# tensorboy/centerpose

Measured on AMD Instinct MI355X. Metric: images/sec end-to-end (backbone+decode), DLA-34 512x512, higher is better.
Workload: dtype f32

## Files before the change

centerpose_amd/csrc/conv3x3_wino24.hip:

```cpp
#include <type_traits>
#include "igemm.h"

#define W24_PH 18
#define W24_PW 18
#define W24_PWP 20
#define W24_KS 16
#define W24_CGS (W24_KS / 4)
#define W24_CG (W24_PH * W24_PWP * 4 + 16)
#define W24_STAGE (W24_CGS * W24_CG)
#define W24_F4 (W24_PH * W24_PW * W24_CGS)
#define W24_SLOTS ((W24_F4 + IG_THREADS - 1) / IG_THREADS)
#define W24_LDR 36
#define W24_RED (16 * 32 * W24_LDR)
#define W24_MAIN (2 * W24_STAGE > W24_RED ? 2 * W24_STAGE : W24_RED)
#define W24_SMEM_FLOATS (W24_MAIN + 16)

typedef float w24_v2 __attribute__((ext_vector_type(2)));
typedef float w24_v4 __attribute__((ext_vector_type(4)));

struct W24Grid {
    int tilesX, tilesY, ntb;
    unsigned mNtb, mTx, mTy;
};
__device__ __forceinline__ int w24_div(int n, int d, unsigned magic) { return d == 1 ? n : (int)__umulhi((unsigned)n, magic); }
__device__ __forceinline__ w24_v4 w24_lds4(const float* p) { return *reinterpret_cast<const w24_v4*>(p); }

__device__ __forceinline__ void w24_output_generic(const ConvArgs& a, float* red, int tid, int b, int y0, int x0, int tile)
{
    const float* const a_res = a.res;
    const bool relu = a.act == CP_ACT_RELU;
    const bool vec_ok = (a.outLd & 3) == 0 && (((size_t)a.out) & 15) == 0 &&
                        (!a_res || ((a.resLd & 3) == 0 && (((size_t)a_res) & 15) == 0));
    const int n4 = tid & 7, n = tile * 32 + n4 * 4;
    const bool nvec = vec_ok && n + 3 < a.Cout;
    w24_v4 sc = {1.f, 1.f, 1.f, 1.f}, sh = {0.f, 0.f, 0.f, 0.f};
    if (nvec) {
        sc = *reinterpret_cast<const w24_v4*>(a.scale + n);
        sh = *reinterpret_cast<const w24_v4*>(a.shift + n);
// ... 104 lines not shown
        const w24_v4 q0 = w24_lds4(rp), q1 = w24_lds4(rp + 128 * W24_LDR), q2 = w24_lds4(rp + 256 * W24_LDR), q3 = w24_lds4(rp + 384 * W24_LDR);
        w24_v4 yv[2];
        yv[0] = (q0 + q1) + q2;
        yv[1] = (q1 - q2) - q3;
#pragma unroll
        for (int aa = 0; aa < 2; ++aa) {
            if (!(okx && oyb + 4 * it + aa < a.H)) continue;
            w24_v4 v = __builtin_elementwise_fma(yv[aa], sc, sh);
            if (a_res) v += rr[it][aa];
            if (relu) v = (w24_v4){cp_relu(v.x), cp_relu(v.y), cp_relu(v.z), cp_relu(v.w)};
            *reinterpret_cast<w24_v4*>(op + (4 * it + aa) * ostep) = v;
        }
    }
}

template <bool FAST>
__device__ __forceinline__ void w24_block(const ConvArgs& a, const W24Grid& gd, int t_, float* smem)
{
    constexpr int CPS = W24_KS / 8;
    const int tid = threadIdx.x, lane = tid & 63, xi = __builtin_amdgcn_readfirstlane(tid >> 6);
    const int h = lane >> 5, m = lane & 31;
    const int NTILES = (a.Cout + 31) >> 5;
    int q_;
    q_ = w24_div(t_, gd.ntb, gd.mNtb); const int nb = t_ - q_ * gd.ntb; t_ = q_;
    q_ = w24_div(t_, gd.tilesX, gd.mTx); const int tx = t_ - q_ * gd.tilesX; t_ = q_;
    q_ = w24_div(t_, gd.tilesY, gd.mTy); const int ty = t_ - q_ * gd.tilesY;
    const int b = q_;
    const int y0 = ty * 16, x0 = tx * 16;
    const int C = a.srcC[0], ld = a.srcLd[0];
    const int KC = C >> 3;
    const float* __restrict__ x = a.src[0];
    const bool interior = y0 >= 1 && y0 + 17 <= a.H && x0 >= 1 && x0 + 17 <= a.W;

    int go[W24_SLOTS], lo[W24_SLOTS];
    bool ok[W24_SLOTS];
#pragma unroll
    for (int s = 0; s < W24_SLOTS; ++s) {
        const int idx = tid + s * IG_THREADS;
        const int pp = idx / W24_CGS, q = idx % W24_CGS;
        const int py = pp / W24_PW, px = pp - py * W24_PW;
        const int gy = y0 - 1 + py, gx = x0 - 1 + px;
        const bool inl = idx < W24_F4;
        ok[s] = inl && gy >= 0 && gy < a.H && gx >= 0 && gx < a.W;
        go[s] = ok[s] ? ((b * a.H + gy) * a.W + gx) * ld + q * 4 : 0;
        lo[s] = inl ? q * W24_CG + (py * W24_PWP + (px ^ ((py >> 1) & 3))) * 4 : -1;
    }
    float4 rg[W24_SLOTS];
    auto stage_load = [&](int c0) __attribute__((always_inline)) {
#pragma unroll
        for (int s = 0; s < W24_SLOTS; ++s) rg[s] = ig_ldg4(x + go[s] + c0);
    };
    auto stage_store = [&](float* buf) __attribute__((always_inline)) {
        if (interior) {
#pragma unroll
            for (int s = 0; s < W24_SLOTS; ++s)
                if ((s + 1) * IG_THREADS <= W24_F4 || lo[s] >= 0) *reinterpret_cast<float4*>(buf + lo[s]) = rg[s];
        } else {
#pragma unroll
            for (int s = 0; s < W24_SLOTS; ++s)
                if ((s + 1) * IG_THREADS <= W24_F4 || lo[s] >= 0) {
                    float4 v = rg[s];
                    if (!ok[s]) v = make_float4(0.f, 0.f, 0.f, 0.f);
// ... 13 lines not shown
    int offA[4], offB[4];
#pragma unroll
    for (int jj = 0; jj < 4; ++jj) { offA[jj] = baseA + ((jj ^ sA) << 2); offB[jj] = baseB + ((jj ^ sB) << 2); }

    int tile = nb;
    if (tile >= NTILES) tile = NTILES - 1;
    const float* ub = a.w + ((size_t)(xi * NTILES + tile) * KC) * 1536 + lane * 4;
    float4 bq[2][6];
    auto load_u = [&](int kc, float4 (&dst)[6]) __attribute__((always_inline)) {
        const int kk = kc < KC ? kc : KC - 1;
#pragma unroll
        for (int nu = 0; nu < 6; ++nu) dst[nu] = ig_ldg4(ub + (size_t)kk * 1536 + nu * 256);
    };

    const int nstage = C / W24_KS;
    stage_load(0);
    load_u(0, bq[0]);
    stage_store(smem);
    if (tid < 4) *reinterpret_cast<float4*>(smem + W24_MAIN + tid * 4) = make_float4(0.f, 0.f, 0.f, 0.f);
    __syncthreads();
    f32x16 acc[6];
    {
        const w24_v4* zp = reinterpret_cast<const w24_v4*>(smem + W24_MAIN);
#pragma unroll
        for (int nu = 0; nu < 6; ++nu)
#pragma unroll
            for (int r4 = 0; r4 < 4; ++r4) {
                w24_v4 z = zp[r4];
                asm volatile("" : "+v"(z));
                acc[nu][4 * r4] = z.x; acc[nu][4 * r4 + 1] = z.y; acc[nu][4 * r4 + 2] = z.z; acc[nu][4 * r4 + 3] = z.w;
            }
    }

// ... 17 lines not shown
                const w24_v2 k4 = {4.f, 4.f}, kn4 = {-4.f, -4.f}, k2 = {2.f, 2.f}, kn2 = {-2.f, -2.f};
                const w24_v2 al = __builtin_elementwise_fma(kn4, tl[2], tl[4]), ah = __builtin_elementwise_fma(kn4, th[2], th[4]);
                const w24_v2 bl = __builtin_elementwise_fma(kn4, tl[1], tl[3]), bh = __builtin_elementwise_fma(kn4, th[1], th[3]);
                const w24_v2 cl = tl[4] - tl[2], chh = th[4] - th[2];
                const w24_v2 fl = tl[3] - tl[1], fh = th[3] - th[1];
                vl[0] = __builtin_elementwise_fma(k4, tl[0] - tl[2], cl); vh[0] = __builtin_elementwise_fma(k4, th[0] - th[2], chh);
                vl[5] = __builtin_elementwise_fma(kn4, fl, tl[5] - tl[3]); vh[5] = __builtin_elementwise_fma(kn4, fh, th[5] - th[3]);
                vl[1] = al + bl; vh[1] = ah + bh;
                vl[2] = al - bl; vh[2] = ah - bh;
                vl[3] = __builtin_elementwise_fma(k2, fl, cl); vh[3] = __builtin_elementwise_fma(k2, fh, chh);
                vl[4] = __builtin_elementwise_fma(kn2, fl, cl); vh[4] = __builtin_elementwise_fma(kn2, fh, chh);
            }
            __builtin_amdgcn_sched_barrier(0);
#pragma unroll
            for (int nu = 0; nu < 6; ++nu) {
                if (nu == 1) {
                    load_u(st * CPS + ch + 1, bq[(ch + 1) & 1]);
                    __builtin_amdgcn_sched_barrier(0);
                }
                if (nu == 3 && ch == 0 && more) {
                    stage_load((st + 1) * W24_KS);
                    __builtin_amdgcn_sched_barrier(0);
                }
                if (nu == 4 && ch == CPS - 1 && more) {
                    stage_store(smem + (BUF ^ 1) * W24_STAGE);
                    __builtin_amdgcn_sched_barrier(0);
                }
                const float4 bb = bq[ch & 1][nu];
                acc[nu] = __builtin_amdgcn_mfma_f32_32x32x2f32(bb.x, vl[nu].x, acc[nu], 0, 0, 0);
                acc[nu] = __builtin_amdgcn_mfma_f32_32x32x2f32(bb.y, vl[nu].y, acc[nu], 0, 0, 0);
                acc[nu] = __builtin_amdgcn_mfma_f32_32x32x2f32(bb.z, vh[nu].x, acc[nu], 0, 0, 0);
                acc[nu] = __builtin_amdgcn_mfma_f32_32x32x2f32(bb.w, vh[nu].y, acc[nu], 0, 0, 0);
            }
            __builtin_amdgcn_sched_barrier(0);
        }
        __syncthreads();
    };
#pragma unroll 1
    for (int st = 0; st < nstage; st += 2) {
        stage(st, std::integral_constant<int, 0>{});
// ... 14 lines not shown

struct W24Group {
    ConvArgs a[4];
    W24Grid gd[4];
    int first[5];
    int n;
};
template <bool FAST>
__global__ __launch_bounds__(IG_THREADS, 2) void conv3x3_wino24_group_kernel(const W24Group g)
{
    extern __shared__ __attribute__((aligned(16))) float smem[];
    const int t = blockIdx.x;
    int k = 0;
    while (k + 1 < g.n && t >= g.first[k + 1]) ++k;
    w24_block<FAST>(g.a[k], g.gd[k], t - g.first[k], smem);
}

static bool w24_fast_epilogue(const ConvArgs& a)
{
    return (a.outLd & 3) == 0 && (a.Cout & 3) == 0 && (((size_t)a.out) & 15) == 0 &&
           (!a.res || ((a.resLd & 3) == 0 && (((size_t)a.res) & 15) == 0)) && (a.act == CP_ACT_NONE || a.act == CP_ACT_RELU) &&
           (long long)a.W * a.outLd * 8 < (1ll << 31) && (long long)a.W * a.resLd * 8 < (1ll << 31);
}

static unsigned w24_magic(int d) { return d <= 1 ? 0u : (unsigned)(((1ull << 32) + (unsigned)d - 1) / (unsigned)d); }

int cp_launch_conv3x3_wino24(const ConvArgs& a, hipStream_t s)
{
    const bool ok = a.nsrc == 1 && a.kh == 3 && a.kw == 3 && a.sy == 1 && a.sx == 1 && a.py == 1 && a.px == 1 &&
                    !a.outNCHW && a.osy == 1 && a.osx == 1 && a.ooy == 0 && a.oox == 0 && a.Ho == a.H && a.Wo == a.W &&
// ... 6 lines not shown
    static CpLdsGuard guard[2];
    {
        const hipError_t e = guard[fast].ensure(fast ? (const void*)conv3x3_wino24_kernel<true> : (const void*)conv3x3_wino24_kernel<false>, smem);
        if (e != hipSuccess) { cp_set_error("conv3x3_winograd24: cannot reserve %d B LDS: %s", smem, hipGetErrorString(e)); return 2; }
    }
    W24Grid gd;
    gd.tilesX = cp_cdiv(a.W, 16); gd.tilesY = cp_cdiv(a.H, 16);
    gd.ntb = (a.Cout + 31) / 32;
    gd.mNtb = w24_magic(gd.ntb); gd.mTx = w24_magic(gd.tilesX); gd.mTy = w24_magic(gd.tilesY);
    const long long grid = (long long)a.B * gd.tilesX * gd.tilesY * gd.ntb;
    const long long dmax = gd.ntb > gd.tilesX ? (gd.ntb > gd.tilesY ? gd.ntb : gd.tilesY) : (gd.tilesX > gd.tilesY ? gd.tilesX : gd.tilesY);
    if (grid * dmax >= (1ll << 32)) { cp_set_error("conv3x3_winograd24: grid %lld too large", grid); return 1; }
    if (fast) hipLaunchKernelGGL(conv3x3_wino24_kernel<true>, dim3((unsigned)grid), dim3(IG_THREADS), smem, s, a, gd);
    else hipLaunchKernelGGL(conv3x3_wino24_kernel<false>, dim3((unsigned)grid), dim3(IG_THREADS), smem, s, a, gd);
    cp_note_kernel(fast ? "conv3x3_wino24_kernel<true>" : "conv3x3_wino24_kernel<false>");
    return 0;
}

int cp_launch_conv3x3_wino24_group(const ConvArgs* a, int n, hipStream_t s)
{
    if (n < 1 || n > 4) { cp_set_error("conv3x3_winograd24_group: 1..4 members (got %d)", n); return 1; }
    W24Group g;
    g.n = n;
    bool fast = true;
    long long total = 0, dmax = 1;
    for (int i = 0; i < n; ++i) {
        const ConvArgs& c = a[i];
        const bool ok = c.nsrc == 1 && c.kh == 3 && c.kw == 3 && c.sy == 1 && c.sx == 1 && c.py == 1 && c.px == 1 &&
                        !c.outNCHW && c.osy == 1 && c.osx == 1 && c.ooy == 0 && c.oox == 0 && c.Ho == c.H && c.Wo == c.W &&
                        c.OH == c.H && c.OW == c.W && c.srcC[0] % 16 == 0 && c.srcLd[0] % 4 == 0 && c.ksplit == 1 &&
// ... 75 lines not shown
```

centerpose_amd/csrc/conv_igemm.hip:

```cpp
#include <cstdlib>
#include "igemm.h"

struct PixSlot {
    int boff;
    int iy0, ix0;
};

template <int BM, int BN, int WAVES_M, int WAVES_N, int MF, bool STEM>
__device__ __forceinline__ void igemm_conv_block(const ConvArgs& a, int tile, int nblocks, float* smem)
{
    using T = IgTile<BM, BN, WAVES_M, WAVES_N, MF>;
    float* As0 = smem;
    float* Bs0 = smem + 2 * T::A_FLOATS;

    const int tid = threadIdx.x, lane = tid & 63, wid = tid >> 6;
    const float* wsub = a.w;
    int pys = a.py, pxs = a.px, ooys = 0, ooxs = 0;
    if (a.nsub > 1) {
        const int per = nblocks / a.nsub, sub = tile / per;
        tile -= sub * per;
        wsub += (size_t)sub * a.ldw * a.K;
        pys -= sub >> 1; pxs -= sub & 1;
        ooys = sub >> 1; ooxs = sub & 1;
    }
// ... 420 lines not shown
                                               float* const* out, void* stream)
{
    CP_CHECK_ARG(d && src && u && scale && shift && res && out && n >= 1 && n <= 4, "conv3x3_winograd24_group: 1..4 members, no null arrays");
    ConvArgs a[4];
    for (int i = 0; i < n; ++i) {
        const float* srcs[1] = {src[i]};
        CP_CHECK_ARG(d[i].nsrc == 1 && !d[i].inNCHW, "conv3x3_winograd24_group: member %d: one NHWC source expected", i);
        if (int rc = conv_args_from_desc(&d[i], srcs, u[i], scale[i], shift[i], res[i], out[i], a[i])) return rc;
        CP_CHECK_ARG(a[i].ksplit == 1, "conv3x3_winograd24_group: no split launches inside a group");
    }
    if (int rc = cp_launch_conv3x3_wino24_group(a, n, (hipStream_t)stream)) return rc;
    CP_CHECK_LAUNCH("conv3x3_wino24_group_kernel");
    return 0;
}

extern "C" int cp_conv3x3_winograd_f32(const cp_conv_desc* d, const float* src, const float* u, const float* scale,
                                       const float* shift, const float* res, float* out, void* stream)
{
    ConvArgs a;
    const float* srcs[1] = {src};
    CP_CHECK_ARG(d && d->nsrc == 1 && !d->inNCHW, "conv3x3_winograd: one NHWC source expected");
    if (int rc = conv_args_from_desc(d, srcs, u, scale, shift, res, out, a)) return rc;
    CP_CHECK_ARG(a.ksplit == 1 || (!res && d->act == CP_ACT_NONE && !d->outNCHW),
                 "conv3x3_winograd: split-C writes raw NHWC partial outputs (no residual, no activation; scale = ones, shift = zeros)");
    const int rc = cp_launch_conv3x3_wino(a, (hipStream_t)stream, d->tile);
    CP_CHECK_ARG(rc >= 0, "conv3x3_winograd: shape not eligible (3x3, stride 1, pad 1, NHWC, C %% 16 == 0)");
    if (rc) return rc;
    CP_CHECK_LAUNCH("conv3x3_wino_kernel");
    return 0;
}
// ... 1 lines not shown
```

centerpose_amd/csrc/igemm.h:

```cpp
#pragma once
#include "common.h"

#define IG_BK 16
#define IG_LDK 20
#define IG_THREADS 256
#define IG_MAX_SRC 4

enum { CP_ACT_NONE = 0, CP_ACT_RELU = 1, CP_ACT_SIGMOID = 2 };

struct ConvArgs {
    const float* src[IG_MAX_SRC];
    int srcC[IG_MAX_SRC];
    int srcLd[IG_MAX_SRC];
    int nsrc, Ctot;
    int B, H, W;
    int Ho, Wo, M;
    int kh, kw, sy, sx, py, px;
    int K;
    const float* w;
    int ldw;
    const float* scale;
    const float* shift;
    const float* res;
    int resLd;
// ... 9 lines not shown
    int omMaskOff;
    int omSigmoid;
    int dily, dilx;
    int ksplit;
    int dg;
    int nsub;
};

int cp_launch_conv3x3_patch(const ConvArgs& a, int in_nchw, hipStream_t s, int variant = 0);
int cp_launch_stem3x3(const ConvArgs& a, hipStream_t s);
int cp_launch_conv3x3_c16(const ConvArgs& a, int in_nchw, hipStream_t s);
int cp_launch_conv3x3_wino(const ConvArgs& a, hipStream_t s, int variant = 0);
int cp_launch_conv3x3_wino24_group(const ConvArgs* a, int n, hipStream_t s);
int cp_launch_head3x3_1x1_w24(const ConvArgs& a, const float* w2, const float* b2, float* out2, int n2, int ld2, int act2, hipStream_t s);
int cp_launch_conv3x3_wino24(const ConvArgs& a, hipStream_t s);
int cp_launch_head3x3_1x1(const ConvArgs& a, const float* w2, const float* b2, float* out2, int n2, int ld2, int act2, hipStream_t s);

int cp_launch_conv_pointwise(const ConvArgs& a, hipStream_t s);
int cp_launch_conv_bf16x3(const ConvArgs& a, int tile, hipStream_t s);

typedef float ig_v4f __attribute__((ext_vector_type(4)));
__device__ __forceinline__ float4 ig_ldg4(const float* p)
{
    const ig_v4f v = *(const __attribute__((address_space(1))) ig_v4f*)(p);
    return make_float4(v.x, v.y, v.z, v.w);
}

__device__ __forceinline__ int ig_xcd_remap(int id, int n)
{
    const int q = n >> 3, r = n & 7, x = id & 7, j = id >> 3;
// ... 212 lines not shown
```

centerpose_amd/csrc/plan_runtime.cpp:

```cpp
#include <cstdio>
#include <cstring>
#include <memory>
#include <string>
#include <vector>
#include "common.h"

extern "C" {
struct cp_conv_desc;
struct cp_dcn_desc;
int cp_abi_version(void);
int cp_conv2d_f32(const cp_conv_desc*, const float* const*, const float*, const float*, const float*, const float*, float*, void*);
int cp_conv3x3_winograd_f32(const cp_conv_desc*, const float*, const float*, const float*, const float*, const float*, float*, void*);
int cp_dcn_v2_f32(const cp_dcn_desc*, const float*, const float*, const float*, const float*, const float*, float*, void*);
int cp_conv3x3_winograd24_group_f32(const cp_conv_desc*, int, const float* const*, const float* const*, const float* const*, const float* const*,
                                    const float* const*, float* const*, void*);
int cp_conv2d_group_f32(const cp_conv_desc*, int, const float* const*, const float* const*, const float* const*, const float* const*,
                        const float* const*, float* const*, void*);
int cp_stem7x7_f32(const float*, const float*, const float*, const float*, float*, int, int, int, int, int, int, int, void*);
int cp_maxpool2d_nhwc_f32(const float*, int, float*, int, int, int, int, int, int, int, int, void*);
int cp_dw_deconv_add_nhwc_f32(const float*, int, const float*, const float*, int, float*, int, int, int, int, int, int, void*);
int cp_sum_up_nhwc_f32(int, const float* const*, const int*, const int*, float*, int, int, int, int, int, int, void*);
int cp_sum_up_group_nhwc_f32(int, const float* const*, const int*, float* const*, int, void*);
int cp_head3x3_1x1_f32(const cp_conv_desc*, const float*, const float*, const float*, const float*, const float*, const float*, float*, int,
                       int, int, void*);
int cp_dwconv2d_nhwc_f32(const float*, int, const float*, const float*, const float*, float*, int, int, int, int, int, int, int, int, int, void*);
int cp_global_avgpool_nhwc_f32(const float*, int, float*, int, int, int, int, void*);
int cp_scale_add_nhwc_f32(const float*, int, const float*, int, const float*, int, float*, int, int, int, int, int, void*);
int cp_shuffle_concat_nhwc_f32(const float*, int, const float*, int, float*, int, long long, int, int, void*);
int cp_multi_pose_decode_f32(const float*, const float*, const float*, const float*, const float*, const float*, int, int, int, int,
                             int, int, float*, float*, int*, void*);
int cp_splitk_reduce_f32(const float*, int, int, int, const float*, const float*, int, float*, int, int, void*);
int cp_sizeof_conv_desc(void);
int cp_sizeof_dcn_desc(void);
int cp_decode_topk_f32(const float*, const float*, int, int, int, int, int, int, float*, int*, void*);
int cp_decode_assign_f32(const float*, const float*, const float*, const float*, const float*, const int*, int, int, int, int, int, float*,
                         void*);
int cp_head_points_f32(const float*, int, const int*, const float*, const float*, const float*, const float*, float*, int, int, int, int, int,
                       int, int, void*);
int cp_flip_merge_pairs_f32(int, const float* const*, float* const*, const int*, int, int, int, int, const int*, void*);
}

namespace {

enum { FN_CONV = 1, FN_WINO = 2, FN_DCN = 3, FN_STEM7 = 4, FN_POOL = 5, FN_UPADD = 6, FN_SUMUP = 7, FN_DWCONV = 8, FN_AVGPOOL = 9,
       FN_SCALEADD = 10, FN_SHUFFLE = 11, FN_HEAD = 12, FN_TOPK = 13, FN_ASSIGN = 14, FN_SPLITK = 15, FN_WINO24G = 16, FN_CONVG = 17, FN_SUMUPG = 18,
       FN_POINTS = 19, FN_FLIPPAIRS = 20 };
enum { REF_NULL = 0, REF_BUF = 1, REF_CONST = 2 };

struct Op {
    uint32_t fn = 0, out_index = 0, stream = 0;
    std::vector<unsigned char> desc;
    std::vector<float*> ptrs;
    std::vector<int> bufid;
    std::vector<int> ints;
};

struct Out { float* p; int shape[4]; int bufid; };

struct ConstPool {
    std::vector<float*> p;
    ~ConstPool() { for (float* q : p) if (q) (void)hipFree(q); }
// ... 82 lines not shown
            return cp_scale_add_nhwc_f32(P[0], I[0], P[1], I[1], P[2], I[2], P[3], I[3], I[4], I[5], I[6], I[7], s);
        case FN_SHUFFLE:
            return cp_shuffle_concat_nhwc_f32(P[0], I[0], P[1], I[1], P[2], I[2], (long long)I[3], I[4], I[5], s);
        case FN_SPLITK:
            return cp_splitk_reduce_f32(P[0], I[0], I[1], I[2], P[1], P[2], I[3], P[3], I[4], I[5], s);
        case FN_TOPK:
            return cp_decode_topk_f32(P[0], P[1], I[0], I[1], I[2], I[3], I[4], I[5], P[2], reinterpret_cast<int*>(P[3]), s);
        case FN_ASSIGN:
            return cp_decode_assign_f32(P[0], P[1], P[2], P[3], P[4], reinterpret_cast<const int*>(P[5]), I[0], I[1], I[2], I[3], I[4], P[6], s);
        case FN_POINTS:
            return cp_head_points_f32(P[0], I[0], reinterpret_cast<const int*>(P[1]), P[2], P[3], P[4], P[5], P[6], I[1], I[2], I[3], I[4], I[5],
                                      I[6], I[7], s);
        case FN_FLIPPAIRS:
            return cp_flip_merge_pairs_f32(I[0], reinterpret_cast<const float* const*>(P.data()), reinterpret_cast<float* const*>(P.data() + 4), I + 5,
                                           I[1], I[2], I[3], I[4], reinterpret_cast<const int*>(P[8]), s);
    }
    cp_set_error("plan: unknown launch function %u", o.fn);
    return 1;
}

bool arity_ok(const Op& o)
{
    switch (o.fn) {
        case FN_CONV: return o.ptrs.size() == 9 && (int)o.desc.size() == cp_sizeof_conv_desc();
        case FN_WINO: return o.ptrs.size() == 6 && (int)o.desc.size() == cp_sizeof_conv_desc();
        case FN_DCN: return o.ptrs.size() == 6 && (int)o.desc.size() == cp_sizeof_dcn_desc();
        case FN_WINO24G: return o.ptrs.size() == 25 && o.ints.size() == 1 && o.ints[0] >= 1 && o.ints[0] <= 4 && (int)o.desc.size() == 4 * cp_sizeof_conv_desc();
        case FN_CONVG: return o.ptrs.size() == 49 && o.ints.size() == 1 && o.ints[0] >= 1 && o.ints[0] <= 8 && (int)o.desc.size() == 8 * cp_sizeof_conv_desc();
        case FN_STEM7: return o.ptrs.size() == 5 && o.ints.size() == 7;
        case FN_POOL: return o.ptrs.size() == 2 && o.ints.size() == 9;
        case FN_UPADD: return o.ptrs.size() == 4 && o.ints.size() == 8;
        case FN_SUMUP: return o.ptrs.size() == 5 && o.ints.size() == 15;
        case FN_SUMUPG: return o.ptrs.size() == 21 && o.ints.size() == 58 && o.ints[0] >= 1 && o.ints[0] <= 4;
        case FN_HEAD: return o.ptrs.size() == 7 && o.ints.size() == 3 && (int)o.desc.size() == cp_sizeof_conv_desc();
        case FN_DWCONV: return o.ptrs.size() == 5 && o.ints.size() == 10;
        case FN_AVGPOOL: return o.ptrs.size() == 2 && o.ints.size() == 5;
        case FN_SCALEADD: return o.ptrs.size() == 4 && o.ints.size() == 8;
        case FN_SHUFFLE: return o.ptrs.size() == 3 && o.ints.size() == 6;
        case FN_SPLITK: return o.ptrs.size() == 4 && o.ints.size() == 6;
        case FN_TOPK: return o.ptrs.size() == 4 && o.ints.size() == 6;
        case FN_ASSIGN: return o.ptrs.size() == 7 && o.ints.size() == 5;
        case FN_POINTS: return o.ptrs.size() == 7 && o.ints.size() == 8;
        case FN_FLIPPAIRS: return o.ptrs.size() == 10 && o.ints.size() == 13 && o.ints[0] >= 1 && o.ints[0] <= 4;
    }
    return false;
}

int run_all(cp_plan* pl, hipStream_t s)
{
    for (const Op& o : pl->ops)
        if (int rc = run_op(o, s)) return rc;
    return 0;
}

struct SchedOp { const Op* op; int stream; int buf_base; };

int run_schedule(const std::vector<SchedOp>& ops, size_t nb, hipStream_t main, hipStream_t side, std::vector<hipEvent_t>& ev)
{
// ... 434 lines not shown
```

centerpose_amd/engine.py:

```python
import os
import warnings
import weakref

import torch

from . import _lib, nets, ops
from .nets import Act


DECODE_TOPK = "decode.nms_topk"
SPARSE_HEADS = ("wh", "hps", "reg", "hp_offset")
FLIP_PEAKS = "flip.merge_peaks"
FLIP_IDX = ((1, 2), (3, 4), (5, 6), (7, 8), (9, 10), (11, 12), (13, 14), (15, 16))


def normalize_state_dict(sd, arch=None):
    out = {}
    for k, v in sd.items():
        if k.startswith("module") and not k.startswith("module_list"):
            k = k[7:]
        out[nets.internal_key(arch, k) if arch is not None else k] = v
    return out


# ... 31 lines not shown
        super().__init__()
        self.dets_only = dets_only
        self.points = None
        self.sd, self.B, self.dev = sd, B, device
        self.const_cache = const_cache if const_cache is not None else {}
        self.pool = BufferPool(device, lambda: len(self.launches))
        if isinstance(sigmoid_heads, bool):
            sigmoid_heads = ("hm", "hm_hp") if sigmoid_heads else ()
        self.sigmoid_heads = tuple(sigmoid_heads)
        self.launches = []
        self.winograd = os.environ.get("CP_WINOGRAD", "1") != "0"
        self.dcn_splitk = os.environ.get("CP_DCN_SPLITK", "1") != "0"
        self.wino_splitc = os.environ.get("CP_WINO_SPLITC", "1") != "0"
        self.conv_splitk = os.environ.get("CP_CONV_SPLITK", "1") != "0"
        self.fuse_heads = os.environ.get("CP_FUSE_HEADS", "1") != "0"
        self._pool_cache = {}
        self.outputs = None

    @property
    def bytes_alloc(self):
        return self.pool.bytes

    def buf(self, H, W, C, split=None):
        Cp = 2 * split[1] if split else ops.round_up(C, 16)
        slot = self.pool.take(self.B * H * W * Cp)
        act = Act(H, W, C, slot[: self.B * H * W * Cp].view(self.B, H, W, Cp), split)
        weakref.finalize(act, self.pool.give, slot)
        return act

    @staticmethod
# ... 178 lines not shown
                outs.append(out)
            self.add("conv", "group:" + chunk[0][1], flops, ops.conv2d_group_launch(recs, slot[:off]))
        return outs

    def emit_maxpool(self, x, k, s, p):
        key = (id(x), k, s, p)
        hit = self._pool_cache.get(key)
        if hit is not None and hit[0]() is x and hit[1]() is not None:
            return hit[1]()
        out = self.buf((x.H + 2 * p - k) // s + 1, (x.W + 2 * p - k) // s + 1, x.C)
        self.add("pool", "maxpool%dx%d" % (k, k), 0, ops.maxpool2d_launch(x.t, out.t, k, s, p))
        self._pool_cache[key] = (weakref.ref(x), weakref.ref(out))
        return out

    def emit_dcn(self, x, conv, bn, co):
        om = self.buf(x.H, x.W, 32)
        wom = ops.pack_conv_weight(self.expand_in(self.w(conv + ".conv_offset_mask.weight"), [x]))
        som, hom = ops.fold_bn(27, None, self.w(conv + ".conv_offset_mask.bias"), self.dev)
        som[27:] = 0.0
        out = self.buf(x.H, x.W, co)
        wp = ops.pack_conv_weight(self.expand_in(self.w(conv + ".weight"), [x]))
        sc, sh = ops.fold_bn(co, self.bn(bn), self.w(conv + ".bias"), self.dev)
        uom = self.wino(wom, x.t.shape[3], 32, key=conv + ".conv_offset_mask", hw=(x.H, x.W))
        if uom is not None:
            self.add_wino(conv + ".conv_offset_mask", 2 * x.H * x.W * 27 * x.C * 9, x.t, wom, uom, som, hom, om.t, 32, ops.ACT_NONE)
        else:
            self.add("conv", conv + ".conv_offset_mask", 2 * x.H * x.W * 27 * x.C * 9,
                     ops.conv2d_launch([x.t], wom, som, hom, om.t, kh=3, kw=3, stride=1, pad=1, cout=32))
        flops = 2 * x.H * x.W * co * x.C * 9
        S = ops.dcn_ksplit(ops.rule_batch(self.B) * x.H * x.W, wp.shape[0]) if self.dcn_splitk else 1
        if S > 1:
            ldw = wp.shape[0]
            ws = self.pool.take(S * self.B * x.H * x.W * ldw)
            wst = ws[: S * self.B * x.H * x.W * ldw].view(S, self.B * x.H * x.W, ldw)
            ones, zeros = self.unit_scale(ldw)
            self.add("dcn", conv, flops, ops.dcn_v2_launch(x.t, om.t, wp, ones, zeros, wst, cout=ldw, om_sigmoid=True, ksplit=S))
            self.add("sum", conv + ".splitk", 0, ops.splitk_reduce_launch(wst, sc, sh, out.t, cout=out.t.shape[3], act=ops.ACT_RELU))
            self.pool.give(ws)
            return out
        self.add("dcn", conv, flops,
                 ops.dcn_v2_launch(x.t, om.t, wp, sc, sh, out.t, cout=out.t.shape[3], om_sigmoid=True, act=ops.ACT_RELU))
        return out

    def emit_up_add(self, x, wname, f, add):
        out = self.buf(x.H * f, x.W * f, x.C)
        wk = ops.pack_dw_deconv_weight(self.w(wname + ".weight"))
        if wk.shape[1] != x.t.shape[3]:
            wk = torch.cat([wk, wk.new_zeros((wk.shape[0], x.t.shape[3] - wk.shape[1]))], 1).contiguous()
        self.add("up", wname, 2 * out.H * out.W * x.C * 4, ops.dw_deconv_add_launch(x.t, wk, add.t, out.t, f))
        return out

    def emit_dwconv(self, x, conv, bn, k, stride, act):
        Ho, Wo = (x.H + 2 * (k // 2) - k) // stride + 1, (x.W + 2 * (k // 2) - k) // stride + 1
        out = self.buf(Ho, Wo, x.C, x.split)
        g, b, mean, var = self.bn(bn)
        scale = g / torch.sqrt(var + ops.BN_EPS)
        shift = b - mean * scale
        wk = ops.pack_dw_weight(self.w(conv + ".weight"))
        wkp = torch.stack([self.expand_vec(row, x) for row in wk], 0).contiguous()
        self.add("dw", conv, 2 * Ho * Wo * x.C * k * k,
                 ops.dwconv2d_launch(x.t, wkp, self.expand_vec(scale, x), self.expand_vec(shift, x), out.t, k, stride, k // 2,
                                     self.act_code(act)))
        return out

# ... 434 lines not shown
        if tuple(images.shape) != tuple(self.input.shape):
            raise ValueError("engine was planned for input %s, got %s" % (tuple(self.input.shape), tuple(images.shape)))
        if images.data_ptr() != self.input.data_ptr():
            self.input.copy_(images)
        if self.use_graph:
            if self.graph is None:
                self.capture()
            self.graph.replay()
        else:
            self.run_eager()
        return self.outputs

    __call__ = forward

    def launch_bytes(self, launches=None):
        grouped = ("cp_conv3x3_winograd24_group_f32", "cp_conv2d_group_f32", "cp_sum_up_group_nhwc_f32", "cp_flip_merge_pairs_f32")
        return [sum(4 * t.numel() for t in (launch.tensors[:-1] if launch.fn in grouped else launch.tensors) if t is not None)
                for _, _, _, launch in (self.launches if launches is None else launches)]

    def profile(self, iters=5):
        torch.cuda.synchronize(self.device)
        self.run_eager()
        nbytes = self.launch_bytes()
        recs = []
        for (kind, name, flops, launch), nb in zip(self.launches, nbytes):
            e0, e1 = torch.cuda.Event(enable_timing=True), torch.cuda.Event(enable_timing=True)
            e0.record()
            for _ in range(iters):
                launch.run()
            e1.record()
            e1.synchronize()
# ... 77 lines not shown
```

centerpose_amd/ops.py:

```python
import ctypes
import os

import torch

from . import _lib

ACT_NONE, ACT_RELU, ACT_SIGMOID, ACT_HSWISH, ACT_HSIGMOID = 0, 1, 2, 3, 4
BN_EPS = 1e-5


class ConvDesc(ctypes.Structure):
    _fields_ = [(n, ctypes.c_int) for n in ("nsrc",)] + [("srcC", ctypes.c_int * 4), ("srcLd", ctypes.c_int * 4)] + \
        [(n, ctypes.c_int) for n in ("B", "H", "W", "Ho", "Wo", "kh", "kw", "sy", "sx", "py", "px", "K", "ldw", "Cout",
                                     "resLd", "outLd", "outNCHW", "OH", "OW", "osy", "osx", "ooy", "oox", "act",
                                     "inNCHW", "tile", "nsub", "ksplit")]


class DcnDesc(ctypes.Structure):
    _fields_ = [(n, ctypes.c_int) for n in ("B", "H", "W", "C", "srcLd", "Ho", "Wo", "kh", "kw", "sy", "sx", "py", "px",
                                            "dily", "dilx", "K", "ldw", "Cout", "omLd", "omSigmoid", "outLd",
                                            "outNCHW", "act", "tile", "ksplit", "dg")]


def round_up(x, m):
# ... 72 lines not shown
    if fn == "cp_shuffle_concat_nhwc_f32":
        return [ptrs[0], ints[0], ptrs[1], ints[1], ptrs[2], ints[2], ctypes.c_longlong(ints[3]), ints[4], ints[5]]
    if fn == "cp_splitk_reduce_f32":
        return [ptrs[0], ints[0], ints[1], ints[2], ptrs[1], ptrs[2], ints[3], ptrs[3], ints[4], ints[5]]
    if fn == "cp_decode_topk_f32":
        return ptrs[:2] + ints + ptrs[2:]
    if fn == "cp_decode_assign_f32":
        return ptrs[:6] + ints + [ptrs[6]]
    if fn == "cp_head_points_f32":
        return [ptrs[0], ints[0]] + ptrs[1:] + ints[1:]
    if fn == "cp_flip_merge_pairs_f32":
        ins = (ctypes.c_void_p * 4)(*[p.value for p in ptrs[:4]])
        outs = (ctypes.c_void_p * 4)(*[p.value for p in ptrs[4:8]])
        meta = (ctypes.c_int * 8)(*ints[5:13])
        return [ints[0], ins, outs, meta] + ints[1:5] + [ptrs[8]]
    raise ValueError("unknown launch function %r" % fn)


FN_IDS = {"cp_conv2d_f32": 1, "cp_conv3x3_winograd_f32": 2, "cp_dcn_v2_f32": 3, "cp_stem7x7_f32": 4,
          "cp_maxpool2d_nhwc_f32": 5, "cp_dw_deconv_add_nhwc_f32": 6, "cp_sum_up_nhwc_f32": 7, "cp_dwconv2d_nhwc_f32": 8,
          "cp_global_avgpool_nhwc_f32": 9, "cp_scale_add_nhwc_f32": 10, "cp_shuffle_concat_nhwc_f32": 11, "cp_head3x3_1x1_f32": 12,
          "cp_decode_topk_f32": 13, "cp_decode_assign_f32": 14, "cp_splitk_reduce_f32": 15, "cp_conv3x3_winograd24_group_f32": 16, "cp_conv2d_group_f32": 17,
          "cp_sum_up_group_nhwc_f32": 18, "cp_head_points_f32": 19,
          "cp_flip_merge_pairs_f32": 20}


def pad_rows(t, ldw):
    Co, K = t.shape
    if Co == ldw:
        return t.contiguous()
    out = torch.zeros((ldw, K), dtype=t.dtype, device=t.device)
    out[:Co] = t
    return out


def pad_vec(v, ldw, fill=0.0):
    out = torch.full((ldw,), fill, dtype=torch.float32, device=v.device)
    out[: v.numel()] = v
    return out
# ... 320 lines not shown
    return out


def pack_dw_deconv_weight(w):
    C, _, k, _ = w.shape
    return w.reshape(C, k * k).t().contiguous().float()


def dw_deconv_add_launch(x, wk, add, out, f):
    B, H, W, C = x.shape
    assert wk.is_contiguous()
    return Launch("cp_dw_deconv_add_nhwc_f32", None, [x, wk, add, out],
                  [_ld(x), _ld(add) if add is not None else 0, _ld(out), B, H, W, C, f])


def dw_deconv_add(x, wk, add, out, f):
    dw_deconv_add_launch(x, wk, add, out, f).run()
    return out


def pack_dw_weight(w):
    C, _, k, _ = w.shape
    return w.reshape(C, k * k).t().contiguous().float()


def dwconv2d_launch(x, wk, scale, shift, out, k, stride, pad, act=ACT_NONE):
    B, H, W, C = x.shape
    assert wk.shape == (k * k, C) and wk.is_contiguous() and scale.numel() >= C and shift.numel() >= C
    return Launch("cp_dwconv2d_nhwc_f32", None, [x, wk, scale, shift, out], [_ld(x), _ld(out), B, H, W, C, k, stride, pad, act])

# ... 162 lines not shown
```

centerpose_amd/plan.py:

```python
import ctypes
import json
import struct

import numpy as np
import torch

from . import _lib, ops

MAGIC = b"CPPLAN04"
MAGIC_V3 = b"CPPLAN03"
MAGIC_V2 = b"CPPLAN02"


def checksum(data):
    mv = memoryview(data).cast("B")
    n = len(mv)
    if n == 0:
        return 2166136261
    buf = (ctypes.c_ubyte * n).from_buffer_copy(mv) if mv.readonly else (ctypes.c_ubyte * n).from_buffer(mv)
    L = _lib.lib()
    L.cp_fnv1a32.restype = ctypes.c_uint32
    L.cp_fnv1a32.argtypes = [ctypes.c_void_p, ctypes.c_size_t]
    return int(L.cp_fnv1a32(ctypes.addressof(buf), n))


REF_NULL, REF_BUF, REF_CONST = 0, 1, 2
FN_NAMES = {v: k for k, v in ops.FN_IDS.items()}
DESC_TYPES = {"cp_conv2d_f32": ops.ConvDesc, "cp_conv3x3_winograd_f32": ops.ConvDesc, "cp_dcn_v2_f32": ops.DcnDesc,
              "cp_conv3x3_winograd24_group_f32": ops.ConvDesc4, "cp_conv2d_group_f32": ops.ConvDesc8,
              "cp_head3x3_1x1_f32": ops.ConvDesc}


def _pad8(b):
    return b + b"\0" * (-len(b) % 8)


def _storage_key(t):
    return t.untyped_storage().data_ptr()


class _Encoder:

    def __init__(self, buffer_storages):
        self.buf_ids = {}
        self.buf_numel = []
# ... 222 lines not shown
```

include/centerpose_hip.h:

```cpp
#ifndef CENTERPOSE_HIP_H
#define CENTERPOSE_HIP_H
#include <stddef.h>
#ifdef __cplusplus
extern "C" {
#endif

int cp_abi_version(void);
const char* cp_target_arch(void);
const char* cp_last_error(void);
const char* cp_last_kernel(void);

enum { CP_ACT_NONE = 0, CP_ACT_RELU = 1, CP_ACT_SIGMOID = 2,
       CP_ACT_HSWISH = 3, CP_ACT_HSIGMOID = 4 };

typedef struct cp_conv_desc {
    int nsrc;
    int srcC[4], srcLd[4];
    int B, H, W;
    int Ho, Wo;
    int kh, kw, sy, sx, py, px;
    int K, ldw;
    int Cout;
    int resLd, outLd;
    int outNCHW;
// ... 11 lines not shown
                        const float* const* shift, const float* const* res, float* const* out, void* stream);

size_t cp_split_bf16_weight_floats(int rows, int K);
int cp_split_bf16_weights_f32(const float* w, int rows, int ldw, int K, float* wb, void* stream);

size_t cp_winograd_weight_floats(int C, int Cout);
int cp_winograd_pack_f32(const float* w, float* u, int C, int Cout, void* stream);
size_t cp_winograd24_weight_floats(int C, int Cout);
int cp_winograd24_pack_f32(const float* w, float* u, int C, int Cout, void* stream);
int cp_conv3x3_winograd_f32(const cp_conv_desc* d, const float* src, const float* u, const float* scale, const float* shift,
                            const float* res, float* out, void* stream);

int cp_conv3x3_winograd24_group_f32(const cp_conv_desc* d, int n, const float* const* src, const float* const* u,
                                    const float* const* scale, const float* const* shift, const float* const* res,
                                    float* const* out, void* stream);

int cp_head3x3_1x1_f32(const cp_conv_desc* d, const float* src, const float* u, const float* scale, const float* shift,
                       const float* w2, const float* b2, float* out2, int n2, int ld2, int act2, void* stream);

typedef struct cp_dcn_desc {
    int B, H, W, C, srcLd;
    int Ho, Wo;
    int kh, kw, sy, sx, py, px, dily, dilx;
    int K, ldw, Cout;
    int omLd, omSigmoid;
    int outLd, outNCHW, act;
    int tile;
    int ksplit;
    int dg;
} cp_dcn_desc;
// ... 78 lines not shown
```

Before: 2179.

## Fuse IDA-up depthwise deconv-add into the following DCN offset-mask Winograd conv

Result: no change. 2199, median of 6 (+0.9%).

```diff
diff --git a/centerpose_amd/csrc/conv3x3_wino24.hip b/centerpose_amd/csrc/conv3x3_wino24.hip
--- a/centerpose_amd/csrc/conv3x3_wino24.hip
+++ b/centerpose_amd/csrc/conv3x3_wino24.hip
@@ -22,6 +22,13 @@
     int tilesX, tilesY, ntb;
     unsigned mNtb, mTx, mTy;
 };
+struct W24NoUp {};
+struct W24Up {
+    const float* proj;
+    const float* wk;
+    float* x;
+    int projLd, Hl, Wl;
+};
 __device__ __forceinline__ int w24_div(int n, int d, unsigned magic) { return d == 1 ? n : (int)__umulhi((unsigned)n, magic); }
 __device__ __forceinline__ w24_v4 w24_lds4(const float* p) { return *reinterpret_cast<const w24_v4*>(p); }
 
@@ -156,8 +163,8 @@
     }
 }
 
-template <bool FAST>
-__device__ __forceinline__ void w24_block(const ConvArgs& a, const W24Grid& gd, int t_, float* smem)
+template <bool FAST, int UPF = 0, class UP = W24NoUp>
+__device__ __forceinline__ void w24_block(const ConvArgs& a, const W24Grid& gd, int t_, float* smem, const UP& up = UP())
 {
     constexpr int CPS = W24_KS / 8;
     const int tid = threadIdx.x, lane = tid & 63, xi = __builtin_amdgcn_readfirstlane(tid >> 6);
@@ -187,7 +194,79 @@
         go[s] = ok[s] ? ((b * a.H + gy) * a.W + gx) * ld + q * 4 : 0;
         lo[s] = inl ? q * W24_CG + (py * W24_PWP + (px ^ ((py >> 1) & 3))) * 4 : -1;
     }
+    constexpr int UF = UPF ? UPF : 1, UK = 2 * UF, PD = 16 / UF + 2, PF4 = PD * PD * W24_CGS, PSLOTS = (PF4 + IG_THREADS - 1) / IG_THREADS;
+    float* const wl = smem + 2 * W24_STAGE;
+    float* const pl = wl + UK * UK * (UPF ? a.srcC[0] : 0);
+    int pk[W24_SLOTS];
+    bool xst[W24_SLOTS];
+    int pgo[PSLOTS];
+    bool pin[PSLOTS];
+    float4 pg[PSLOTS];
+    if constexpr (UPF != 0) {
+#pragma unroll
+        for (int s = 0; s < W24_SLOTS; ++s) {
+            const int idx = tid + s * IG_THREADS;
+            const int pp = idx / W24_CGS, q = idx % W24_CGS;
+            const int py = pp / W24_PW, px = pp - py * W24_PW;
+            const int ay = py - 1 + UF / 2, ax = px - 1 + UF / 2;
+            pk[s] = (lo[s] >> 2 & 0x7ff) | (((q * PD + ay / UF + 1) * PD + ax / UF + 1) << 11) | ((((ay % UF) * UK + ax % UF) * 4 + q) << 20);
+            xst[s] = ok[s] && py >= 1 && py <= 16 && px >= 1 && px <= 16;
+        }
+#pragma unroll
+        for (int k = 0; k < PSLOTS; ++k) {
+            const int j = tid + k * IG_THREADS;
+            const int q = j % W24_CGS, pix = j / W24_CGS;
+            const int pr = pix / PD, pc = pix - pr * PD;
+            const int ly = y0 / UF - 1 + pr, lx = x0 / UF - 1 + pc;
+            pin[k] = j < PF4 && ly >= 0 && ly < up.Hl && lx >= 0 && lx < up.Wl;
+            pgo[k] = pin[k] ? ((b * up.Hl + ly) * up.Wl + lx) * up.projLd + q * 4 : 0;
+        }
+    }
+    auto p_load = [&](int c0) __attribute__((always_inline)) {
+        if constexpr (UPF != 0) {
+#pragma unroll
+            for (int k = 0; k < PSLOTS; ++k) {
+                int g = pgo[k];
+                asm volatile("" : "+v"(g));
+                pg[k] = ig_ldg4(up.proj + g + c0);
+            }
+        }
+    };
+    auto p_store = [&](float* pb) __attribute__((always_inline)) {
+#pragma unroll
+        for (int k = 0; k < PSLOTS; ++k) {
+            const int j = tid + k * IG_THREADS;
+            if (j < PF4) *reinterpret_cast<float4*>(pb + ((j % W24_CGS) * PD * PD + j / W24_CGS) * 4) = pin[k] ? pg[k] : make_float4(0.f, 0.f, 0.f, 0.f);
+        }
+    };
     float4 rg[W24_SLOTS];
+    auto up_store = [&](float* buf, const float* pb, int st) __attribute__((always_inline)) {
+        const float* wst = wl + st * (UK * UK * 16);
+        if constexpr (UPF != 0)
+#pragma unroll
+        for (int s = 0; s < W24_SLOTS; ++s)
+            if ((s + 1) * IG_THREADS <= W24_F4 || tid + s * IG_THREADS < W24_F4) {
+                w24_v4 acc = {0.f, 0.f, 0.f, 0.f};
+                int pks = pk[s];
+                asm volatile("" : "+v"(pks));
+#pragma unroll
+                for (int ty = 0; ty < 2; ++ty)
+#pragma unroll
+                    for (int tx = 0; tx < 2; ++tx) {
+                        const w24_v4 v = w24_lds4(pb + (pks >> 11 & 0x1ff) * 4 - (ty * PD + tx) * 4);
+                        const w24_v4 ww = w24_lds4(wst + (pks >> 20) * 4 + (ty * UF * UK + tx * UF) * 16);
+                        acc = __builtin_elementwise_fma(v, ww, acc);
+                    }
+                acc += (w24_v4){rg[s].x, rg[s].y, rg[s].z, rg[s].w};
+                if (!ok[s]) acc = (w24_v4){0.f, 0.f, 0.f, 0.f};
+                *reinterpret_cast<w24_v4*>(buf + (pks & 0x7ff) * 4) = acc;
+                if (xst[s]) {
+                    int g = go[s];
+                    asm volatile("" : "+v"(g));
+                    *reinterpret_cast<w24_v4*>(up.x + g + st * W24_KS) = acc;
+                }
+            }
+    };
     auto stage_load = [&](int c0) __attribute__((always_inline)) {
 #pragma unroll
         for (int s = 0; s < W24_SLOTS; ++s) rg[s] = ig_ldg4(x + go[s] + c0);
@@ -231,9 +310,27 @@
     };
 
     const int nstage = C / W24_KS;
+    if constexpr (UPF != 0) {
+        const int C4 = C >> 2;
+        for (int j = tid; j < UK * UK * C4; j += IG_THREADS) {
+            const int tap = j / C4, c4 = j - tap * C4;
+            *reinterpret_cast<float4*>(wl + ((c4 >> 2) * UK * UK + tap) * 16 + (c4 & 3) * 4) = ig_ldg4(up.wk + (size_t)tap * C + c4 * 4);
+        }
+        p_load(0);
+        p_store(pl);
+        if (nstage > 1) {
+            p_load(W24_KS);
+            p_store(pl + PF4 * 4);
+        }
+        stage_load(0);
+        load_u(0, bq[0]);
+        __syncthreads();
+        up_store(smem, pl, 0);
+    } else {
     stage_load(0);
     load_u(0, bq[0]);
     stage_store(smem);
+    }
     if (tid < 4) *reinterpret_cast<float4*>(smem + W24_MAIN + tid * 4) = make_float4(0.f, 0.f, 0.f, 0.f);
     __syncthreads();
     f32x16 acc[6];
@@ -281,6 +378,16 @@
             __builtin_amdgcn_sched_barrier(0);
 #pragma unroll
             for (int nu = 0; nu < 6; ++nu) {
+                if constexpr (UPF != 0) {
+                    if (nu == 0 && ch == 0 && st + 2 < nstage) {
+                        p_load((st + 2) * W24_KS);
+                        __builtin_amdgcn_sched_barrier(0);
+                    }
+                    if (nu == 3 && ch == 0 && st + 2 < nstage) {
+                        p_store(pl + BUF * (PF4 * 4));
+                        __builtin_amdgcn_sched_barrier(0);
+                    }
+                }
                 if (nu == 1) {
                     load_u(st * CPS + ch + 1, bq[(ch + 1) & 1]);
                     __builtin_amdgcn_sched_barrier(0);
@@ -290,7 +397,11 @@
                     __builtin_amdgcn_sched_barrier(0);
                 }
                 if (nu == 4 && ch == CPS - 1 && more) {
+                    if constexpr (UPF != 0) {
+                        up_store(smem + (BUF ^ 1) * W24_STAGE, pl + (BUF ^ 1) * (PF4 * 4), st + 1);
+                    } else {
                     stage_store(smem + (BUF ^ 1) * W24_STAGE);
+                    }
                     __builtin_amdgcn_sched_barrier(0);
                 }
                 const float4 bb = bq[ch & 1][nu];
@@ -335,6 +446,13 @@
     int k = 0;
     while (k + 1 < g.n && t >= g.first[k + 1]) ++k;
     w24_block<FAST>(g.a[k], g.gd[k], t - g.first[k], smem);
+}
+
+template <int UPF>
+__global__ __launch_bounds__(IG_THREADS, 2) void idaup_node_wino24_kernel(const ConvArgs a, const W24Grid gd, const W24Up up)
+{
+    extern __shared__ __attribute__((aligned(16))) float smem[];
+    w24_block<true, UPF, W24Up>(a, gd, ig_xcd_remap(blockIdx.x, gridDim.x), smem, up);
 }
 
 static bool w24_fast_epilogue(const ConvArgs& a)
@@ -371,6 +489,39 @@
     if (fast) hipLaunchKernelGGL(conv3x3_wino24_kernel<true>, dim3((unsigned)grid), dim3(IG_THREADS), smem, s, a, gd);
     else hipLaunchKernelGGL(conv3x3_wino24_kernel<false>, dim3((unsigned)grid), dim3(IG_THREADS), smem, s, a, gd);
     cp_note_kernel(fast ? "conv3x3_wino24_kernel<true>" : "conv3x3_wino24_kernel<false>");
+    return 0;
+}
+
+int cp_launch_idaup_node_wino24(const ConvArgs& a, const float* proj, int projLd, const float* wk, float* x, int f, hipStream_t s)
+{
+    const int C = a.srcC[0];
+    const bool ok = a.nsrc == 1 && a.kh == 3 && a.kw == 3 && a.sy == 1 && a.sx == 1 && a.py == 1 && a.px == 1 &&
+                    !a.outNCHW && a.osy == 1 && a.osx == 1 && a.ooy == 0 && a.oox == 0 && a.Ho == a.H && a.Wo == a.W &&
+                    a.OH == a.H && a.OW == a.W && C % 16 == 0 && a.srcLd[0] % 4 == 0 && a.srcLd[0] >= C && a.ksplit == 1 &&
+                    (f == 2 || f == 4) && a.H % f == 0 && a.W % f == 0 && projLd % 4 == 0 && projLd >= C &&
+                    (((size_t)a.src[0] | (size_t)a.w | (size_t)proj | (size_t)wk | (size_t)x) & 15) == 0 &&
+                    (long long)a.B * a.H * a.W * a.srcLd[0] < (1ll << 31) && (long long)a.B * (a.H / f) * (a.W / f) * projLd < (1ll << 31) &&
+                    a.Cout <= 32 && !a.res && w24_fast_epilogue(a) &&
+                    4 * f * f * C + 2 * (16 / f + 2) * (16 / f + 2) * 16 <= W24_RED - 2 * W24_STAGE;
+    if (!ok) return -1;
+    const int smem = W24_SMEM_FLOATS * 4;
+    static CpLdsGuard guard[2];
+    {
+        const hipError_t e = guard[f == 4].ensure(f == 4 ? (const void*)idaup_node_wino24_kernel<4> : (const void*)idaup_node_wino24_kernel<2>, smem);
+        if (e != hipSuccess) { cp_set_error("idaup_node: cannot reserve %d B LDS: %s", smem, hipGetErrorString(e)); return 2; }
+    }
+    W24Grid gd;
+    gd.tilesX = cp_cdiv(a.W, 16); gd.tilesY = cp_cdiv(a.H, 16);
+    gd.ntb = 1;
+    gd.mNtb = w24_magic(gd.ntb); gd.mTx = w24_magic(gd.tilesX); gd.mTy = w24_magic(gd.tilesY);
+    const long long grid = (long long)a.B * gd.tilesX * gd.tilesY;
+    const long long dmax = gd.tilesX > gd.tilesY ? gd.tilesX : gd.tilesY;
+    if (grid * dmax >= (1ll << 32)) { cp_set_error("idaup_node: grid %lld too large", grid); return 1; }
+    W24Up up;
+    up.proj = proj; up.wk = wk; up.x = x; up.projLd = projLd; up.Hl = a.H / f; up.Wl = a.W / f;
+    if (f == 4) hipLaunchKernelGGL(idaup_node_wino24_kernel<4>, dim3((unsigned)grid), dim3(IG_THREADS), smem, s, a, gd, up);
+    else hipLaunchKernelGGL(idaup_node_wino24_kernel<2>, dim3((unsigned)grid), dim3(IG_THREADS), smem, s, a, gd, up);
+    cp_note_kernel(f == 4 ? "idaup_node_wino24_kernel<4>" : "idaup_node_wino24_kernel<2>");
     return 0;
 }
 
diff --git a/centerpose_amd/csrc/conv_igemm.hip b/centerpose_amd/csrc/conv_igemm.hip
--- a/centerpose_amd/csrc/conv_igemm.hip
+++ b/centerpose_amd/csrc/conv_igemm.hip
@@ -458,6 +458,20 @@
     return 0;
 }
 
+extern "C" int cp_idaup_node_winograd24_f32(const cp_conv_desc* d, const float* skip, const float* proj, const float* wk, const float* u,
+                                            const float* scale, const float* shift, float* x, float* om, int projLd, int f, void* stream)
+{
+    ConvArgs a;
+    const float* srcs[1] = {skip};
+    CP_CHECK_ARG(d && d->nsrc == 1 && !d->inNCHW && proj && wk && x, "idaup_node: one NHWC skip map, proj, taps and x expected");
+    if (int rc = conv_args_from_desc(d, srcs, u, scale, shift, nullptr, om, a)) return rc;
+    const int rc = cp_launch_idaup_node_wino24(a, proj, projLd, wk, x, f, (hipStream_t)stream);
+    CP_CHECK_ARG(rc >= 0, "idaup_node: shape not eligible (f = 2 / 4, H, W %% f == 0, C %% 16 == 0, <= 32 dense NHWC output channels, taps fit in LDS)");
+    if (rc) return rc;
+    CP_CHECK_LAUNCH("idaup_node_wino24_kernel");
+    return 0;
+}
+
 extern "C" int cp_conv3x3_winograd_f32(const cp_conv_desc* d, const float* src, const float* u, const float* scale,
                                        const float* shift, const float* res, float* out, void* stream)
 {
diff --git a/centerpose_amd/csrc/igemm.h b/centerpose_amd/csrc/igemm.h
--- a/centerpose_amd/csrc/igemm.h
+++ b/centerpose_amd/csrc/igemm.h
@@ -47,6 +47,7 @@
 int cp_launch_conv3x3_wino24_group(const ConvArgs* a, int n, hipStream_t s);
 int cp_launch_head3x3_1x1_w24(const ConvArgs& a, const float* w2, const float* b2, float* out2, int n2, int ld2, int act2, hipStream_t s);
 int cp_launch_conv3x3_wino24(const ConvArgs& a, hipStream_t s);
+int cp_launch_idaup_node_wino24(const ConvArgs& a, const float* proj, int projLd, const float* wk, float* x, int f, hipStream_t s);
 int cp_launch_head3x3_1x1(const ConvArgs& a, const float* w2, const float* b2, float* out2, int n2, int ld2, int act2, hipStream_t s);
 
 int cp_launch_conv_pointwise(const ConvArgs& a, hipStream_t s);
diff --git a/centerpose_amd/csrc/plan_runtime.cpp b/centerpose_amd/csrc/plan_runtime.cpp
--- a/centerpose_amd/csrc/plan_runtime.cpp
+++ b/centerpose_amd/csrc/plan_runtime.cpp
@@ -38,13 +38,15 @@
 int cp_head_points_f32(const float*, int, const int*, const float*, const float*, const float*, const float*, float*, int, int, int, int, int,
                        int, int, void*);
 int cp_flip_merge_pairs_f32(int, const float* const*, float* const*, const int*, int, int, int, int, const int*, void*);
+int cp_idaup_node_winograd24_f32(const cp_conv_desc*, const float*, const float*, const float*, const float*, const float*, const float*, float*,
+                                 float*, int, int, void*);
 }
 
 namespace {
 
 enum { FN_CONV = 1, FN_WINO = 2, FN_DCN = 3, FN_STEM7 = 4, FN_POOL = 5, FN_UPADD = 6, FN_SUMUP = 7, FN_DWCONV = 8, FN_AVGPOOL = 9,
        FN_SCALEADD = 10, FN_SHUFFLE = 11, FN_HEAD = 12, FN_TOPK = 13, FN_ASSIGN = 14, FN_SPLITK = 15, FN_WINO24G = 16, FN_CONVG = 17, FN_SUMUPG = 18,
-       FN_POINTS = 19, FN_FLIPPAIRS = 20 };
+       FN_POINTS = 19, FN_FLIPPAIRS = 20, FN_IDAUPNODE = 21 };
 enum { REF_NULL = 0, REF_BUF = 1, REF_CONST = 2 };
 
 struct Op {
@@ -157,6 +159,9 @@
         case FN_FLIPPAIRS:
             return cp_flip_merge_pairs_f32(I[0], reinterpret_cast<const float* const*>(P.data()), reinterpret_cast<float* const*>(P.data() + 4), I + 5,
                                            I[1], I[2], I[3], I[4], reinterpret_cast<const int*>(P[8]), s);
+        case FN_IDAUPNODE:
+            return cp_idaup_node_winograd24_f32(reinterpret_cast<const cp_conv_desc*>(o.desc.data()), P[0], P[1], P[2], P[3], P[4], P[5], P[6], P[7],
+                                                I[0], I[1], s);
     }
     cp_set_error("plan: unknown launch function %u", o.fn);
     return 1;
@@ -185,6 +190,7 @@
         case FN_ASSIGN: return o.ptrs.size() == 7 && o.ints.size() == 5;
         case FN_POINTS: return o.ptrs.size() == 7 && o.ints.size() == 8;
         case FN_FLIPPAIRS: return o.ptrs.size() == 10 && o.ints.size() == 13 && o.ints[0] >= 1 && o.ints[0] <= 4;
+        case FN_IDAUPNODE: return o.ptrs.size() == 9 && o.ints.size() == 2 && (int)o.desc.size() == cp_sizeof_conv_desc();
     }
     return false;
 }
diff --git a/centerpose_amd/engine.py b/centerpose_amd/engine.py
--- a/centerpose_amd/engine.py
+++ b/centerpose_amd/engine.py
@@ -69,6 +69,8 @@
         self.wino_splitc = os.environ.get("CP_WINO_SPLITC", "1") != "0"
         self.conv_splitk = os.environ.get("CP_CONV_SPLITK", "1") != "0"
         self.fuse_heads = os.environ.get("CP_FUSE_HEADS", "1") != "0"
+        self.idaup_fuse = os.environ.get("CP_IDAUP_FUSE", "1") != "0"
+        self._last_up = None
         self._pool_cache = {}
         self.outputs = None
 
@@ -277,7 +279,9 @@
         return out
 
     def emit_dcn(self, x, conv, bn, co):
-        om = self.buf(x.H, x.W, 32)
+        up, self._last_up = self._last_up, None
+        fuse = up is not None and up["out"] is x and up["index"] == len(self.launches) - 1
+        om = Act(x.H, x.W, 32, up["om"], parent=x.parent) if fuse else self.buf(x.H, x.W, 32)
         wom = ops.pack_conv_weight(self.expand_in(self.w(conv + ".conv_offset_mask.weight"), [x]))
         som, hom = ops.fold_bn(27, None, self.w(conv + ".conv_offset_mask.bias"), self.dev)
         som[27:] = 0.0
@@ -285,7 +289,12 @@
         wp = ops.pack_conv_weight(self.expand_in(self.w(conv + ".weight"), [x]))
         sc, sh = ops.fold_bn(co, self.bn(bn), self.w(conv + ".bias"), self.dev)
         uom = self.wino(wom, x.t.shape[3], 32, key=conv + ".conv_offset_mask", hw=(x.H, x.W))
-        if uom is not None:
+        if fuse:
+            assert isinstance(uom, tuple)
+            _, upname, upflops, _ = self.launches.pop()
+            self.add("wino24", "%s.conv_offset_mask+%s" % (conv, upname.rsplit(".", 1)[-1]), upflops // self.B + 2 * x.H * x.W * 27 * x.C * 9,
+                     ops.idaup_node_launch(up["proj"].t, up["wk"], up["add"].t, x.t, uom[1], wom, som, hom, om.t, up["f"], up["whole"]))
+        elif uom is not None:
             self.add_wino(conv + ".conv_offset_mask", 2 * x.H * x.W * 27 * x.C * 9, x.t, wom, uom, som, hom, om.t, 32, ops.ACT_NONE)
         else:
             self.add("conv", conv + ".conv_offset_mask", 2 * x.H * x.W * 27 * x.C * 9,
@@ -305,12 +314,29 @@
                  ops.dcn_v2_launch(x.t, om.t, wp, sc, sh, out.t, cout=out.t.shape[3], om_sigmoid=True, act=ops.ACT_RELU))
         return out
 
+    def idaup_fusable(self, x, f, add):
+        Cp, H, W = x.t.shape[3], x.H * f, x.W * f
+        return self.idaup_fuse and self.winograd and not x.split and not add.split and add.t.shape[3] == Cp and ops.idaup_node_eligible(Cp, f) and \
+            ops.wino_eligible(Cp, 3, 1, 1, 1) and ops.wino24_wanted(self.B, H, W, Cp, 32)
+
     def emit_up_add(self, x, wname, f, add):
-        out = self.buf(x.H * f, x.W * f, x.C)
+        fusable = self.idaup_fusable(x, f, add)
+        if fusable:
+            Cp, H, W = x.t.shape[3], x.H * f, x.W * f
+            nx, nom = self.B * H * W * Cp, self.B * H * W * 32
+            slot = self.pool.take(nx + nom)
+            holder = Act(1, 1, 1, slot)
+            weakref.finalize(holder, self.pool.give, slot)
+            out = Act(H, W, x.C, slot[:nx].view(self.B, H, W, Cp), parent=holder)
+        else:
+            out = self.buf(x.H * f, x.W * f, x.C)
         wk = ops.pack_dw_deconv_weight(self.w(wname + ".weight"))
         if wk.shape[1] != x.t.shape[3]:
             wk = torch.cat([wk, wk.new_zeros((wk.shape[0], x.t.shape[3] - wk.shape[1]))], 1).contiguous()
         self.add("up", wname, 2 * out.H * out.W * x.C * 4, ops.dw_deconv_add_launch(x.t, wk, add.t, out.t, f))
+        if fusable:
+            self._last_up = dict(index=len(self.launches) - 1, out=out, proj=x, wk=wk, add=add, f=f, whole=slot[:nx + nom],
+                                 om=slot[nx:nx + nom].view(self.B, H, W, 32))
         return out
 
     def emit_dwconv(self, x, conv, bn, k, stride, act):
@@ -775,7 +801,8 @@
     __call__ = forward
 
     def launch_bytes(self, launches=None):
-        grouped = ("cp_conv3x3_winograd24_group_f32", "cp_conv2d_group_f32", "cp_sum_up_group_nhwc_f32", "cp_flip_merge_pairs_f32")
+        grouped = ("cp_conv3x3_winograd24_group_f32", "cp_conv2d_group_f32", "cp_sum_up_group_nhwc_f32", "cp_flip_merge_pairs_f32",
+                   "cp_idaup_node_winograd24_f32")
         return [sum(4 * t.numel() for t in (launch.tensors[:-1] if launch.fn in grouped else launch.tensors) if t is not None)
                 for _, _, _, launch in (self.launches if launches is None else launches)]
 
diff --git a/centerpose_amd/ops.py b/centerpose_amd/ops.py
--- a/centerpose_amd/ops.py
+++ b/centerpose_amd/ops.py
@@ -110,6 +110,8 @@
         outs = (ctypes.c_void_p * 4)(*[p.value for p in ptrs[4:8]])
         meta = (ctypes.c_int * 8)(*ints[5:13])
         return [ints[0], ins, outs, meta] + ints[1:5] + [ptrs[8]]
+    if fn == "cp_idaup_node_winograd24_f32":
+        return [d] + ptrs[:8] + ints
     raise ValueError("unknown launch function %r" % fn)
 
 
@@ -118,7 +120,7 @@
           "cp_global_avgpool_nhwc_f32": 9, "cp_scale_add_nhwc_f32": 10, "cp_shuffle_concat_nhwc_f32": 11, "cp_head3x3_1x1_f32": 12,
           "cp_decode_topk_f32": 13, "cp_decode_assign_f32": 14, "cp_splitk_reduce_f32": 15, "cp_conv3x3_winograd24_group_f32": 16, "cp_conv2d_group_f32": 17,
           "cp_sum_up_group_nhwc_f32": 18, "cp_head_points_f32": 19,
-          "cp_flip_merge_pairs_f32": 20}
+          "cp_flip_merge_pairs_f32": 20, "cp_idaup_node_winograd24_f32": 21}
 
 
 def pad_rows(t, ldw):
@@ -469,6 +471,20 @@
                   [_ld(x), _ld(add) if add is not None else 0, _ld(out), B, H, W, C, f])
 
 
+def idaup_node_eligible(C, f):
+    return f in (2, 4) and C % 16 == 0 and 4 * f * f * C + 2 * (16 // f + 2) ** 2 * 16 <= 6784
+
+
+def idaup_node_launch(proj, wk, skip, x, u24, wp, scale, shift, om, f, whole):
+    B, H, W, C = skip.shape
+    assert tuple(proj.shape) == (B, H // f, W // f, C) and H % f == 0 and W % f == 0 and idaup_node_eligible(C, f)
+    assert tuple(x.shape) == (B, H, W, C) and _ld(x) == _ld(skip) and tuple(wk.shape) == (4 * f * f, C) and wk.is_contiguous()
+    assert all(t.untyped_storage().data_ptr() == whole.untyped_storage().data_ptr() for t in (x, om))
+    assert skip.untyped_storage().data_ptr() != whole.untyped_storage().data_ptr()
+    d = conv2d_launch([skip], wp, scale, shift, om, kh=3, kw=3, stride=1, pad=1, cout=om.shape[3], wino=u24, tile=WINO24).desc
+    return Launch("cp_idaup_node_winograd24_f32", d, [skip, proj, wk, u24, scale, shift, x, om, whole], [_ld(proj), f])
+
+
 def dw_deconv_add(x, wk, add, out, f):
     dw_deconv_add_launch(x, wk, add, out, f).run()
     return out
diff --git a/centerpose_amd/plan.py b/centerpose_amd/plan.py
--- a/centerpose_amd/plan.py
+++ b/centerpose_amd/plan.py
@@ -28,7 +28,7 @@
 FN_NAMES = {v: k for k, v in ops.FN_IDS.items()}
 DESC_TYPES = {"cp_conv2d_f32": ops.ConvDesc, "cp_conv3x3_winograd_f32": ops.ConvDesc, "cp_dcn_v2_f32": ops.DcnDesc,
               "cp_conv3x3_winograd24_group_f32": ops.ConvDesc4, "cp_conv2d_group_f32": ops.ConvDesc8,
-              "cp_head3x3_1x1_f32": ops.ConvDesc}
+              "cp_head3x3_1x1_f32": ops.ConvDesc, "cp_idaup_node_winograd24_f32": ops.ConvDesc}
 
 
 def _pad8(b):
diff --git a/include/centerpose_hip.h b/include/centerpose_hip.h
--- a/include/centerpose_hip.h
+++ b/include/centerpose_hip.h
@@ -49,6 +49,9 @@
 int cp_conv3x3_winograd24_group_f32(const cp_conv_desc* d, int n, const float* const* src, const float* const* u,
                                     const float* const* scale, const float* const* shift, const float* const* res,
                                     float* const* out, void* stream);
+
+int cp_idaup_node_winograd24_f32(const cp_conv_desc* d, const float* skip, const float* proj, const float* wk, const float* u,
+                                 const float* scale, const float* shift, float* x, float* om, int projLd, int f, void* stream);
 
 int cp_head3x3_1x1_f32(const cp_conv_desc* d, const float* src, const float* u, const float* scale, const float* shift,
                        const float* w2, const float* b2, float* out2, int n2, int ld2, int act2, void* stream);
```
